# NVIDIA/vid2vid

Measured on AMD Instinct MI355X. Metric: synthesized frames/sec (Vid2VidModelG.inference, 512x256), higher is better.
Workload: dtype bf16; 1 GPU; label2city 512x256 inference, n_scales_spatial=1, --fg --use_instance, ngf=128 n_blocks=9 (411.3M params random-init, 2115 GFLOP/frame as dense convolutions, of which the 2 one-hot label stems (266 GFLOP dense) run as exact weight gather-sums), batch 1 per sequence, 1 sequence per GPU; launches_per_frame=113, hipgraph=True, graph_lanes=3, paired_launches=True, tile_selection=profiles/tune_cache.json, world_size=1, parallelism=replicas x1 (independent sequences, no collective), output_finite=True

## Files before the change

### include/v2v_hip.h

```cpp
#ifndef V2V_HIP_H
#define V2V_HIP_H

#include <stdint.h>

#ifdef __cplusplus
extern "C" {
#endif

#define V2V_EINVAL (-1)

#define V2V_F32  0
#define V2V_BF16 1

#define V2V_PAD_ZERO    0
#define V2V_PAD_REFLECT 1

#define V2V_ACT_NONE    0
#define V2V_ACT_RELU    1
#define V2V_ACT_LEAKY   2
#define V2V_ACT_TANH    3
#define V2V_ACT_SIGMOID 4

#define V2V_OUT_RAW_F32_NHWC 0
#define V2V_OUT_ACT_NHWC     1
// ... 17 lines not shown
    int32_t stride;
    int32_t pad;
    int32_t pad_mode;
    int32_t transposed;
    int32_t OH, OW;
    int32_t dtype;
    int32_t out_mode;
    int32_t act;
    float   act_param;
    float   out_scale;
    int32_t tile;
    int32_t* fin_counter;
    const float* fin_gamma;
    const float* fin_beta;
    float*  fin_scale_shift;
    float*  fin_running_mean;
    float*  fin_running_var;
    float   fin_eps;
    float   fin_momentum;
    int64_t fin_count;
    int32_t splitk;
    int32_t prefetch;
    void*   slabs;
    int32_t* sk_counter;
    int32_t w_korder;
    int32_t ablate;
    const void* res0;
    const void* res1;
    int32_t act_split;
    int32_t act_b;
    float   act_param_b;
    float   out_scale_b;
    double* fin_workspace;
} v2v_conv_desc;


#define V2V_FIN_TAG_WORD (256 + 64 * 128 + 256)




int64_t v2v_conv_packed_elems(int32_t cin, int32_t cin_stride, int32_t cout, int32_t KH, int32_t KW,
                              int32_t transposed, int32_t stride, int32_t pad, int32_t dtype);
int     v2v_conv_pack_weights(const float* w, void* dst, int32_t cin, int32_t cin_stride, int32_t cout,
                              int32_t KH, int32_t KW, int32_t transposed, int32_t stride, int32_t pad,
                              int32_t dtype, int32_t korder, void* stream);

int     v2v_conv_stats_rows(const v2v_conv_desc* d);
int     v2v_conv_stats_rows_per_sample(const v2v_conv_desc* d);
int64_t v2v_conv_splitk_workspace(const v2v_conv_desc* d, int32_t* tickets);
int     v2v_conv_fused_norm_max_workgroups(void);
int     v2v_fastdiv_magic(uint32_t d, uint32_t* m_out, int32_t* l_out);
int     v2v_conv_tile_config(const v2v_conv_desc* d);
#define V2V_TILE_FAMILY_IGEMM   0
#define V2V_TILE_FAMILY_PATCH   1
#define V2V_TILE_FAMILY_PP      2
#define V2V_TILE_FAMILY_PP2     3
#define V2V_TILE_FAMILY_PP3     4
#define V2V_TILE_FAMILY_S7      5
#define V2V_TILE_FAMILY_S2      6
#define V2V_TILE_FAMILY_T2      7
#define V2V_TILE_FAMILY_ONE     8
#define V2V_TILE_FAMILY_T2_ONE  9
#define V2V_TILE_FAMILY_HEAD    10
#define V2V_TILE_FAMILY_C8      11
#define V2V_TILE_FAMILY_ROWSUM  12
#define V2V_TILE_GROUPED        1
// ... 341 lines not shown
```

### vid2vid_amd/csrc/conv3x3_t2_kernel.h

```cpp
#pragma once
#include "conv3x3_pp3_kernel.h"

namespace v2v {

namespace t2k {
constexpr int CLS[9] = {3, 3, 3, 3, 1, 1, 2, 2, 0};
constexpr int KK[9]  = {0, 2, 6, 8, 3, 5, 1, 7, 4};
constexpr int DY[9]  = {1, 1, 0, 0, 0, 0, 1, 0, 0};
constexpr int DX[9]  = {1, 0, 1, 0, 1, 0, 0, 0, 0};
}

template <typename T, int TH, int TW, int BN, int D>
__global__ __launch_bounds__(512) void conv3x3_t2_kernel(const ConvKArgs p) {
    constexpr int VEC = ElemTraits<T>::VEC;
    constexpr int NW = 8, WGM = 4, WGN = 2, SS = 4;
    constexpr int BM = TH * TW;
    constexpr int PW = TW + 1, PR = (TH + 1) * PW;
    constexpr int NG = (PR + 7) / 8;
    constexpr int GP = (NG + NW - 1) / NW;
    constexpr int PATCH = GP * NW * 1024;
    constexpr int BST = BN * 128;
    constexpr int LB = BN / 8 / NW;
    constexpr int NPT = 9 - D;
    constexpr int PPT = (GP + NPT - 1) / NPT;
// ... 180 lines not shown
        static_for<NDMA - DMA_IN_SLOTS>([&](auto dc) { dma(std::integral_constant<int, DMA_IN_SLOTS + decltype(dc)::value>{}); });
        wait_vmcnt<pp3::pending_at(TAP, GP, LB, D)>();
        asm volatile("s_waitcnt lgkmcnt(0)" ::: "memory");
        stage = nstage;
        if constexpr (TAP == 8) {
            ++cc;
            const char* t = pa; pa = pn; pn = const_cast<char*>(t);
        }
    };
    auto chunk = [&](auto par0c) {
        constexpr int P0 = decltype(par0c)::value;
        iteration(std::integral_constant<int, 0>{}, std::integral_constant<int, P0>{});
        iteration(std::integral_constant<int, 1>{}, std::integral_constant<int, 1 - P0>{});
        iteration(std::integral_constant<int, 2>{}, std::integral_constant<int, P0>{});
        iteration(std::integral_constant<int, 3>{}, std::integral_constant<int, 1 - P0>{});
        iteration(std::integral_constant<int, 4>{}, std::integral_constant<int, P0>{});
        iteration(std::integral_constant<int, 5>{}, std::integral_constant<int, 1 - P0>{});
        iteration(std::integral_constant<int, 6>{}, std::integral_constant<int, P0>{});
        iteration(std::integral_constant<int, 7>{}, std::integral_constant<int, 1 - P0>{});
        iteration(std::integral_constant<int, 8>{}, std::integral_constant<int, P0>{});
    };
    int c = 0;
    for (; c + 1 < ncc; c += 2) {
        chunk(std::integral_constant<int, 0>{});
        chunk(std::integral_constant<int, 1>{});
    }
    if (c < ncc) chunk(std::integral_constant<int, 0>{});
    (void)nsteps;

    asm volatile("s_waitcnt vmcnt(0)" ::: "memory");
    __syncthreads();

    const int OH = p.OH, OW = p.OW;
    static_for<4>([&](auto cc_) {
        constexpr int CL = decltype(cc_)::value;
        auto pix_of = [&](int row) -> int {
            const int oy = 2 * (a0 + row / TW) + (CL >> 1), ox = 2 * (b0 + (row & (TW - 1))) + (CL & 1);
            if (oy >= OH || ox >= OW) return -1;
            return (n_img * OH + oy) * OW + ox;
        };
        conv_epilogue<T, BM, BN, WGM, WGN, false>(p, acc[CL], smem, tid, wm, wn, false, CL, tiles, lin, 0, 1, nt, CL * p.m_tiles + mt, pix_of);
        __syncthreads();
    });
}

template <typename T, int TH, int TW, int BN, int D>
static int launch_t2_cfg(const ConvKArgs& k, hipStream_t s) {
    constexpr int NW = 8;
    constexpr int GP = (((TH + 1) * (TW + 1) + 7) / 8 + NW - 1) / NW;
    const size_t lds = (size_t)2 * GP * NW * 1024 + (size_t)D * BN * 128;
    auto kern = conv3x3_t2_kernel<T, TH, TW, BN, D>;
    static bool attr_done = false;
    if (!attr_done) {
        (void)hipFuncSetAttribute(reinterpret_cast<const void*>(kern), hipFuncAttributeMaxDynamicSharedMemorySize, (int)lds);
        attr_done = true;
    }
    dim3 grid((unsigned)(k.m_tiles * k.n_tiles), 1u, 1u);
    hipLaunchKernelGGL(kern, grid, dim3(NW * 64), lds, s, k);
    return check_launch();
}

template <typename T>
static inline int launch_t2_typed(int cfg, const ConvKArgs& k, hipStream_t s) {
    switch (cfg) {
        case 110: return launch_t2_cfg<T, V2V_TILE_GEOM(110), 4>(k, s);
        case 111: return launch_t2_cfg<T, V2V_TILE_GEOM(111), 4>(k, s);
        case 112: return launch_t2_cfg<T, V2V_TILE_GEOM(112), 4>(k, s);
        case 113: return launch_t2_cfg<T, V2V_TILE_GEOM(113), 3>(k, s);
    }
    set_error("conv: unknown transposed stride-2 patch tile config %d", cfg);
    return V2V_EINVAL;
}

}
// ... 1 lines not shown
```

### vid2vid_amd/csrc/conv_igemm.hip

```cpp
#include "conv3x3_pp_kernel.h"
#include "conv3x3_pp2_kernel.h"
#include "conv3x3_pp3_kernel.h"
#include "conv3x3_s2_kernel.h"
#include "conv3x3_t2_kernel.h"
#include "conv7x7_head_kernel.h"
#include <cstdarg>
#include <cstring>
#include <cstdlib>
#include <algorithm>

namespace v2v {

static int bke_of(int dtype) { return dtype == V2V_BF16 ? 64 : 32; }

static void convt_axis(int K, int pad, int stride, int par, int* k0, int* nk, int* d0) {
    if (stride == 1) { *k0 = 0; *nk = K; *d0 = pad; return; }
    *k0 = (par + pad) & 1;
    *nk = (*k0 < K) ? (K - *k0 + 1) / 2 : 0;
    *d0 = (par + pad - *k0) / 2;
}

struct ConvGeom {
    int ncls;
    int nkh[4], nkw[4], kh0[4], kw0[4], dh0[4], dw0[4], ktot[4], kpad[4];
// ... 516 lines not shown
        break;
    case V2V_TILE_FAMILY_HEAD:
        if (d->transposed || d->KH != 7 || d->KW != 7 || d->stride != 1 || d->pad != 3 || d->cout > 32 ||
            d->cin_stride % (bke_of(d->dtype) / 2) != 0 || d->w_korder != 0 || d->splitk > 1 || d->fin_counter ||
            !(d->out_mode == V2V_OUT_F32_NCHW || d->out_mode == V2V_OUT_RAW_F32_NHWC) ||
            (d->stats && d->out_mode != V2V_OUT_RAW_F32_NHWC) || in_bytes >= (1ll << 32)) {
            set_error("conv: tile config 60 (7x7, cout <= 32) needs a 7x7/s1/p3 Conv2d, cin_stride %% %d == 0 (whole 64-byte half chunks), planar fp32 or raw "
                      "NHWC output without in-kernel norm finalize", bke_of(d->dtype) / 2); return V2V_EINVAL;
        }
        break;
    case V2V_TILE_FAMILY_S7:
        if (d->transposed || d->KH != 7 || d->KW != 7 || d->stride != 1 || d->pad != 3 ||
            d->cin_stride % bke_of(d->dtype) != 0 || d->w_korder != 1 || d->out_mode == V2V_OUT_NORM_ACT_NHWC ||
            (d->pad_mode == V2V_PAD_REFLECT && (d->H <= 3 || d->W <= 3)) || in_bytes >= (1ll << 32)) {
            set_error("conv: tile config %d needs a bf16 7x7/s1/p3 Conv2d, cin_stride %% %d == 0, korder-1 weights, no fused norm",
                      t->id, bke_of(d->dtype)); return V2V_EINVAL;
        }
        break;
    case V2V_TILE_FAMILY_T2: case V2V_TILE_FAMILY_T2_ONE:
        if (!d->transposed || d->KH != 3 || d->KW != 3 || d->stride != 2 || d->pad != 1 ||
            d->cin_stride % bke_of(d->dtype) != 0 || d->w_korder != 2 || d->splitk > 1 || d->out_mode == V2V_OUT_NORM_ACT_NHWC ||
            in_bytes >= (1ll << 32)) {
            set_error("conv: transposed stride-2 patch tile config %d needs a ConvTranspose2d(3x3, s2, p1), cin_stride %% %d == 0, korder-2 weights, no split-K",
                      t->id, bke_of(d->dtype)); return V2V_EINVAL;
        }
        if (fam == V2V_TILE_FAMILY_T2_ONE && (d->cin_stride != 64 || d->cout > t->bn || (d->cout & 3) || (d->cout_stride & 3) || ((unsigned long long)d->out & 15ull) ||
                               (d->out_mode != V2V_OUT_RAW_F32_NHWC && d->out_mode != V2V_OUT_RAW_ACT_NHWC) || d->fin_workspace != nullptr || d->H % t->th != 0 || d->W % t->tw != 0 ||
                               d->OH != 2 * d->H || d->OW != 2 * d->W)) {
            set_error("conv: tile config %d (persistent transposed stride-2 tile) needs bf16, cin_stride 64, cout <= %d and %% 4 == 0, raw fp32 NHWC output (16-byte aligned "
                      "rows), no two-level finalize workspace, H %% %d == 0, W %% %d == 0, OH = 2 H, OW = 2 W", t->id, t->bn, t->th, t->tw);
            return V2V_EINVAL;
        }
        k.woff[0] = 0; k.wrow[0] = 9 * d->cin_stride;
        k.fin_rows = (t->flags & V2V_TILE_PERSISTENT) ? 0 : 4 * k.m_tiles;
        break;
    case V2V_TILE_FAMILY_S2:
        if (d->transposed || d->KH != 3 || d->KW != 3 || d->stride != 2 || d->pad != 1 || d->pad_mode != V2V_PAD_ZERO ||
            d->cin_stride % bke_of(d->dtype) != 0 || d->w_korder != 1 || d->splitk > 1 || d->out_mode == V2V_OUT_NORM_ACT_NHWC ||
            in_bytes >= (1ll << 32)) {
            set_error("conv: stride-2 patch tile config %d needs a 3x3/s2/p1 zero-padded Conv2d, cin_stride %% %d == 0, korder-1 weights, no split-K",
                      t->id, bke_of(d->dtype)); return V2V_EINVAL;
        }
        break;
    case V2V_TILE_FAMILY_PATCH: case V2V_TILE_FAMILY_PP: case V2V_TILE_FAMILY_PP2: case V2V_TILE_FAMILY_PP3: case V2V_TILE_FAMILY_ONE: {
        const bool pad2_ok = d->pad == 2 && (t->flags & V2V_TILE_PAD2) && d->pad_mode == V2V_PAD_ZERO && d->out_mode != V2V_OUT_NORM_ACT_NHWC;
        if (d->transposed || d->KH != 3 || d->KW != 3 || d->stride != 1 || (d->pad != 1 && !pad2_ok) ||
            d->cin_stride % bke_of(d->dtype) != 0 || d->w_korder != 1 || in_bytes >= (1ll << 32)) {
            set_error("conv: patch tile config %d needs a 3x3/s1/p1 Conv2d, cin_stride %% %d == 0 and korder-1 weights",
                      t->id, bke_of(d->dtype)); return V2V_EINVAL;
        }
        if (fam == V2V_TILE_FAMILY_ONE && (((t->flags & V2V_TILE_EXACT_BN) && d->cout != t->bn) || d->cout > t->bn || (d->cout & 3) || (d->cout_stride & 3) || ((unsigned long long)d->out & 15ull) ||
                               (d->out_mode != V2V_OUT_RAW_F32_NHWC && d->out_mode != V2V_OUT_RAW_ACT_NHWC) || d->fin_workspace != nullptr || d->OH % t->th != 0 || d->OW % t->tw != 0)) {
            set_error("conv: tile configs 140 - 143 (persistent, weights resident) need cout <= %d (143: exactly) and %% 4 == 0, raw fp32 NHWC output (16-byte aligned rows), "
                      "no two-level finalize workspace, OH %% %d == 0 and OW %% %d == 0", t->bn, t->th, t->tw);
            return V2V_EINVAL;
        }
        if ((t->flags & V2V_TILE_SINGLE_CHUNK) && (d->cin_stride != bke_of(d->dtype) || d->splitk > 1 || d->out_mode == V2V_OUT_NORM_ACT_NHWC)) {
            set_error("conv: tile config %d is a single-chunk tile: bf16, cin_stride exactly %d, no split-K, no fused norm", t->id, bke_of(d->dtype));
            return V2V_EINVAL;
        }
        break;
    }
    default:
        if (d->w_korder != 0) { set_error("conv: tile config %d reads tap-major (korder 0) weights", t->id); return V2V_EINVAL; }
    }
    if (fam != V2V_TILE_FAMILY_IGEMM && k.tiles_h > 0 && k.tiles_w > 0 && k.m_tiles > 0) {
        const uint32_t dv[3] = {(uint32_t)k.m_tiles, (uint32_t)(k.tiles_h * k.tiles_w), (uint32_t)k.tiles_w};
        for (int i = 0; i < 3; ++i) {
            uint32_t m = 0; int32_t l = 0;
            if (v2v_fastdiv_magic(dv[i], &m, &l) != 0) return V2V_EINVAL;
            k.idx_m[i] = m; k.idx_l[i] = l;
        }
    }
    k.splitk = d->splitk > 1 ? d->splitk : 1;
    int nk_min = k.kpad[0] / bke_of(d->dtype);
    for (int cc = 1; cc < g.ncls; ++cc) nk_min = std::min(nk_min, k.kpad[cc] / bke_of(d->dtype));
    if (fam != V2V_TILE_FAMILY_IGEMM) nk_min = 2 * (d->cin_stride / bke_of(d->dtype));
    if (k.splitk > 1 && (k.splitk > 16 || nk_min / k.splitk < 2)) {
        set_error("conv: splitk %d needs >= 2 K chunks per slice (layer has %d)", k.splitk, nk_min); return V2V_EINVAL;
    }
    op->sk_tickets = g.ncls * k.m_tiles * k.n_tiles;
    op->slab_bytes = k.splitk > 1 ? (long long)op->sk_tickets * k.splitk * t->bm * t->bn * 4 : 0;
    if (k.splitk > 1) {
        if (launching && (!d->slabs || !d->sk_counter)) { set_error("conv: splitk needs slabs and sk_counter"); return V2V_EINVAL; }
        k.slabs = (float*)d->slabs; k.sk_counter = d->sk_counter;
    }
    if (d->fin_counter && d->fin_workspace && d->out_mode != V2V_OUT_NORM_ACT_NHWC) {
        const int rows = k.fin_rows > 0 ? k.fin_rows : g.ncls * k.m_tiles;
        const int groups = rows > 512 ? (rows >= 64 * 128 ? 64 : (rows + 127) / 128) : 0;
        if (groups > 0) {
            if (k.n_tiles > 128) { set_error("conv: two-level finalize supports up to 128 channel tiles"); return V2V_EINVAL; }
            k.fin_groups = groups; k.fin_ws = d->fin_workspace;
        }
    }
    k.ablate = d->ablate;
    k.dbg = g_conv_dbg_clocks;
    {
        static const int rev = [] { const char* e = getenv("V2V_CLS_ORDER"); return (e && e[0] == '0') ? 0 : 1; }();
        k.cls_rev = rev;
    }
    k.pf_dist = (d->prefetch > 0 && (t->flags & V2V_TILE_HELPER)) ? d->prefetch : 0;
    {
        static const int ep_fast = [] { const char* e = getenv("V2V_EPILOGUE_FAST"); return (e && e[0] == '0') ? 0 : 1; }();
        k.ep_slow = ep_fast ? 0 : 1;
    }
    k.pf_mask = (k.pf_dist > 0 && k.m_tiles >= 8) ? 3 : 0;
    return 0;
}

}

using namespace v2v;

extern "C" int64_t v2v_conv_packed_elems(int32_t cin, int32_t cin_stride, int32_t cout, int32_t KH, int32_t KW,
                                         int32_t transposed, int32_t stride, int32_t pad, int32_t dtype) {
    (void)cin;
    ConvGeom g;
    conv_geom(cin_stride, cout, KH, KW, transposed, stride, pad, dtype, &g);
    return g.total;
}

extern "C" int v2v_conv_pack_weights(const float* w, void* dst, int32_t cin, int32_t cin_stride, int32_t cout,
                                     int32_t KH, int32_t KW, int32_t transposed, int32_t stride, int32_t pad,
                                     int32_t dtype, int32_t korder, void* stream) {
    if (!w || !dst) { set_error("pack: null pointer"); return V2V_EINVAL; }
// ... 18 lines not shown
    conv_geom(cin_stride, cout, KH, KW, (korder == 4 || korder == 5) ? 0 : transposed, stride, pad, dtype, &g);
    int kh0_flip = -1;
    if (korder == 4) { kh0_flip = KH - 1; korder = 1; }
    if (korder == 5) { kh0_flip = KH - 1; korder = 0; }
    if (korder == 2) {
        g.ncls = 1; g.nkh[0] = 3; g.nkw[0] = 3; g.kh0[0] = 0; g.kw0[0] = 0;
        g.ktot[0] = g.kpad[0] = g.wrow[0] = 9 * cin_stride; g.woff[0] = 0;
        g.total = (long long)g.cout_p * g.wrow[0];
        stride = 1;
        korder = 1;
    }
    auto op = std::make_unique<PackOp>();
    PackArgs& a = op->a;
    a.w = w; a.dst = dst; a.cin = cin; a.cin_stride = cin_stride; a.cout = cout; a.cout_p = g.cout_p;
    a.KH = KH; a.KW = KW; a.transposed = transposed; a.kstep = stride; a.ncls = g.ncls; a.total = g.total; a.dtype = dtype;
    a.korder = korder; a.bke = bke_of(dtype); a.src_cl = src_cl;
    for (int c = 0; c < 4; ++c) {
        a.nkh[c] = g.nkh[c]; a.nkw[c] = g.nkw[c]; a.kh0[c] = g.kh0[c]; a.kw0[c] = g.kw0[c];
        a.kpad[c] = g.kpad[c]; a.wrow[c] = g.wrow[c]; a.woff[c] = g.woff[c];
    }
    if (kh0_flip >= 0) { a.kh0[0] = kh0_flip; a.kw0[0] = KW - 1; a.kstep = -1; }
    return submit(std::move(op), stream);
}

extern "C" int v2v_conv_debug_clocks(void* device_buffer) {
    g_conv_dbg_clocks = reinterpret_cast<unsigned long long*>(device_buffer);
    return 0;
}

extern "C" int v2v_conv_stats_rows(const v2v_conv_desc* d) {
    ConvOp op;
    if (build_conv(d, &op, false) != 0) return V2V_EINVAL;
    if (op.tile->flags & V2V_TILE_PERSISTENT) return one_grid(op.k.m_tiles * op.k.n_tiles, device_cus());
    return op.ncls * op.k.m_tiles;
}

extern "C" int v2v_conv_stats_rows_per_sample(const v2v_conv_desc* d) {
    ConvOp op;
    if (build_conv(d, &op, false) != 0) return V2V_EINVAL;
    if ((op.tile->flags & V2V_TILE_PERSISTENT) || op.ncls != 1 || d->N <= 0) return 0;
    if (op.tile->family == V2V_TILE_FAMILY_IGEMM) {
        const long long hw = (long long)d->OH * d->OW;
        return hw % op.tile->bm == 0 ? (int)(hw / op.tile->bm) : 0;
    }
    return op.k.m_tiles / d->N;
}

extern "C" int64_t v2v_conv_splitk_workspace(const v2v_conv_desc* d, int32_t* tickets) {
    ConvOp op;
    if (build_conv(d, &op, false) != 0) return V2V_EINVAL;
    if (tickets) *tickets = op.sk_tickets;
    return op.slab_bytes;
}

extern "C" int v2v_conv_tile_count(void) { return kNumConvTiles; }

extern "C" int v2v_conv_tile_info(int32_t index, struct v2v_conv_tile_info* out) {
    if (index < 0 || index >= kNumConvTiles || !out) { set_error("conv tile info: index %d outside [0, %d)", index, kNumConvTiles); return V2V_EINVAL; }
    const ConvTile& t = kConvTiles[index];
    *out = {t.id, t.family, t.bm, t.bn, t.th, t.tw, t.korder, t.flags};
    return 0;
}

extern "C" int v2v_conv_tile_config(const v2v_conv_desc* d) {
    ConvOp op;
    if (build_conv(d, &op, false) != 0) return V2V_EINVAL;
    return op.tile->id;
}


extern "C" int v2v_fastdiv_magic(uint32_t d, uint32_t* m_out, int32_t* l_out) {
    if (d == 0 || d >= (1u << 31) || !m_out || !l_out) { set_error("fastdiv: divisor out of range"); return V2V_EINVAL; }
// ... 84 lines not shown
```

### vid2vid_amd/csrc/conv_igemm_kernel.h

```cpp
#pragma once
#include "v2v_internal.h"
#include "conv_tiles.h"

namespace v2v {

struct ConvGroupPtrs {
    const char* in; const char* w; const float* bias; char* out; float* stats;
    int* fin_counter; const float* fin_gamma; const float* fin_beta; float* fin_out; float* fin_rmean; float* fin_rvar;
    float* slabs; int* sk_counter;
    const char* res0; const char* res1;
};

struct ConvKArgs {
    const char* in;
    const char* w;
    const char* zero_page;
    const float* bias;
    char* out;
    float* stats;
    int N, H, W, cin_stride;
    int cout, cout_stride, cout_p;
    int OH, OW;
    int sm;
    int os;
    int pad_mode;
    int Mc[4], OHc[4], OWc[4];
    int m_tiles, n_tiles;
    int out_mode, act;
    float act_param, out_scale;
    int nkh[4], nkw[4];
    int dh0[4], dw0[4];
    int dstep;
    int ktot[4], kpad[4], wrow[4];
    long long woff[4];
    int* fin_counter; const float* fin_gamma; const float* fin_beta; float* fin_out;
    float* fin_rmean; float* fin_rvar;
    float fin_eps, fin_momentum; double fin_inv_count, fin_unbias;
    int splitk; float* slabs; int* sk_counter;
    int pf_dist, pf_mask;
    int tiles_h, tiles_w;
    int ablate;
    int cls_rev;
    int act_split, act_b; float act_param_b, out_scale_b;
    const char* res0; const char* res1;
    unsigned div_m[4][2]; int div_l[4][2];
    int* status;
    ConvGroupPtrs g1;
    int fin_groups; double* fin_ws;
    int fin_rows;
    unsigned long long* dbg;
    int grp_xcd;
    int ep_slow;
    unsigned idx_m[3]; int idx_l[3];
    int pair_x;
};

#ifndef V2V_STAMP_MASK
#define V2V_STAMP_MASK 0
#endif
#define V2V_STAMP(p_, k_)                                                                                                   \
    do {                                                                                                                   \
        if (((V2V_STAMP_MASK >> (k_)) & 1) && (p_).dbg != nullptr && threadIdx.x == 0)                                                                       \
            (p_).dbg[((size_t)(blockIdx.z * gridDim.y + blockIdx.y) * gridDim.x + blockIdx.x) * 8 + (k_)] = wall_clock64(); \
    } while (0)

__device__ __forceinline__ int xcd_remap(int bid, int ntot) {
    const int q = ntot >> 3, r = ntot & 7, xcd = bid & 7, idx = bid >> 3;
    return (xcd < r ? xcd * (q + 1) : r * (q + 1) + (xcd - r) * q) + idx;
}

__device__ __forceinline__ int grouped_xcd_map(int bx, int bz, int ntot, int& member) {
    const int xcd = bx & 7;
    const int idx = (bx >> 3) + bz * (ntot >> 3);
    member = xcd >> 2;
    return (xcd & 3) * (ntot >> 2) + idx;
}

__device__ __forceinline__ int fast_div(int n, unsigned M, int l) { return (int)((__umulhi(M, (unsigned)n) + (unsigned)n) >> l); }

__device__ __forceinline__ void patch_tile_index(const ConvKArgs& p, const int lin_all, int& lin, int& slice, int& nt, int& mt,
                                                 int& n_img, int& th, int& tw) {
    const int S = p.splitk;
// ... 20 lines not shown
}

template <int N> __device__ __forceinline__ void wait_vmcnt() {
    asm volatile("s_waitcnt vmcnt(%0)" ::"n"(N) : "memory");
}

__device__ __forceinline__ void mfma_results_ready() {
    asm volatile("s_nop 7\n\ts_nop 7\n\ts_nop 2" ::: "memory");
    __builtin_amdgcn_sched_barrier(0);
}

template <typename T> struct Mma;
template <> struct Mma<bf16_t> {
    typedef bf16x8 Frag;
    __device__ static __forceinline__ void run(const Frag& a, const Frag& b, f32x16& c) {
        c = __builtin_amdgcn_mfma_f32_32x32x16_bf16(a, b, c, 0, 0, 0);
    }
};
template <> struct Mma<float> {
    typedef f32x4 Frag;
    __device__ static __forceinline__ void run(const Frag& a, const Frag& b, f32x16& c) {
        c = __builtin_amdgcn_mfma_f32_32x32x2f32(a[0], b[0], c, 0, 0, 0);
        c = __builtin_amdgcn_mfma_f32_32x32x2f32(a[1], b[1], c, 0, 0, 0);
        c = __builtin_amdgcn_mfma_f32_32x32x2f32(a[2], b[2], c, 0, 0, 0);
        c = __builtin_amdgcn_mfma_f32_32x32x2f32(a[3], b[3], c, 0, 0, 0);
    }
};

template <typename T, int BM, int BN, int WGM, int WGN, bool FUSED_NORM = false, typename PixOf = void>
__device__ __forceinline__ void conv_epilogue(const ConvKArgs& p, f32x16 (&acc)[BM / WGM / 32][BN / WGN / 32], char* smem,
                                              const int tid, const int wm, const int wn, const bool helper,
                                              const int cls, const int tiles, const int lin, const int slice, const int S,
                                              const int nt, const int stat_row, PixOf pix_of, const bool tile_full = false,
                                              const unsigned fin_epoch = 0u) {
    constexpr int WM = BM / WGM, WN = BN / WGN;
    constexpr int TM = WM / 32, TN = WN / 32;
    constexpr int NW = WGM * WGN;
    const int lane = tid & 63;
    const int lr = lane & 31, hi = lane >> 5;
    if (S > 1) {
        constexpr int NT = NW * 64;
        constexpr unsigned SLAB = (unsigned)BM * BN * 4u;
        typedef __attribute__((ext_vector_type(4))) unsigned u32x4;
        const long long tile_id = (long long)cls * tiles + lin;
        char* const sbase = reinterpret_cast<char*>(p.slabs) + tile_id * (long long)S * SLAB;
        const __amdgpu_buffer_rsrc_t rsrc = __builtin_amdgcn_make_buffer_rsrc(sbase, 0, (int)(S * SLAB), 0x00020000);
        if (!helper) {
            const unsigned my = (unsigned)slice * SLAB + (unsigned)tid * 16u;
#pragma unroll
            for (int i = 0; i < TM; ++i)
#pragma unroll
                for (int j = 0; j < TN; ++j)
#pragma unroll
                    for (int q = 0; q < 4; ++q) {
                        u32x4 v;
                        v[0] = __float_as_uint(acc[i][j][4 * q + 0]); v[1] = __float_as_uint(acc[i][j][4 * q + 1]);
                        v[2] = __float_as_uint(acc[i][j][4 * q + 2]); v[3] = __float_as_uint(acc[i][j][4 * q + 3]);
                        __builtin_amdgcn_raw_buffer_store_b128(v, rsrc, my + (unsigned)(((i * TN + j) * 4 + q) * NT * 16), 0, 16);
                    }
        }
        asm volatile("s_waitcnt vmcnt(0)" ::: "memory");
        __syncthreads();
        int* flag = reinterpret_cast<int*>(smem + 16384);
        if (tid == 0) {
            int* cnt = p.sk_counter + tile_id;
            const int tk = __hip_atomic_fetch_add(cnt, 1, __ATOMIC_RELAXED, __HIP_MEMORY_SCOPE_AGENT);
            const int last = tk == S - 1 ? 1 : 0;
// ... 421 lines not shown
            for (int i = 0; i < TM; ++i)
#pragma unroll
                for (int r = 0; r < 16; ++r)
                    if (opx[i][r] >= 0) {
                        const unsigned n = (unsigned)opx[i][r] / ohow;
                        opx[i][r] = (int)(n * (unsigned)p.cout * ohow + ((unsigned)opx[i][r] - n * ohow));
                    }
        }
#pragma unroll
        for (int j = 0; j < TN; ++j) {
            const int ncol = nt * BN + wn * WN + j * 32 + lr;
            const bool nvalid = ncol < p.cout && !helper;
            const float bv = (p.bias != nullptr && nvalid) ? p.bias[ncol] : 0.f;
#pragma unroll
            for (int i = 0; i < TM; ++i)
#pragma unroll
                for (int r = 0; r < 16; ++r)
                    if (opx[i][r] >= 0 && nvalid)
                        out[(unsigned)opx[i][r] + (unsigned)ncol * ohow] = apply_act(acc[i][j][r] + bv, e_act, e_act_param) * e_out_scale;
        }
    }
    V2V_STAMP(p, 4);
    if (want_stats) {
        __syncthreads();
        if (tid < BN) {
            const int ncol = nt * BN + tid;
            if (ncol < p.cout) {
                float s1 = 0.f, s2 = 0.f;
#pragma unroll
                for (int q = 0; q < WGM; ++q) {
                    s1 += red[(q * BN + tid) * 2 + 0];
                    s2 += red[(q * BN + tid) * 2 + 1];
                }
                float* dst = p.stats + ((long long)stat_row * p.cout + ncol) * 2;
                if (p.fin_counter != nullptr) {
                    const unsigned long long bits = (unsigned long long)__float_as_uint(s1) |
                                                    ((unsigned long long)__float_as_uint(s2) << 32);
                    __hip_atomic_store(reinterpret_cast<unsigned long long*>(dst), bits, __ATOMIC_RELAXED,
                                       __HIP_MEMORY_SCOPE_AGENT);
                } else {
                    dst[0] = s1;
                    dst[1] = s2;
                }
            }
        }
        if (p.fin_counter != nullptr) {
            asm volatile("s_waitcnt vmcnt(0)" ::: "memory");
            __syncthreads();
            V2V_STAMP(p, 5);
            int* flag = reinterpret_cast<int*>(smem + 16384);
            const int total = p.fin_rows > 0 ? p.fin_rows : (int)gridDim.y * p.m_tiles;
            constexpr int NT = NW * 64;
            if (p.fin_groups > 0) {
                const int G = p.fin_groups;
                int g = (int)(((long long)stat_row * G) / total);
                while ((int)(((long long)total * (g + 1)) / G) <= stat_row) ++g;
                while ((int)(((long long)total * g) / G) > stat_row) --g;
                const int r0 = (int)(((long long)total * g) / G), r1 = (int)(((long long)total * (g + 1)) / G);
                if (tid == 0) {
                    int* cnt = p.fin_counter + 256 + g * p.n_tiles + nt;
                    const int tk = __hip_atomic_fetch_add(cnt, 1, __ATOMIC_RELAXED, __HIP_MEMORY_SCOPE_AGENT);
                    const int last = tk == (r1 - r0) - 1 ? 1 : 0;
                    if (last) __hip_atomic_store(cnt, 0, __ATOMIC_RELAXED, __HIP_MEMORY_SCOPE_AGENT);
                    *flag = last;
                }
                __syncthreads();
                if (!*flag) { V2V_STAMP(p, 6); return; }
                __syncthreads();
                double* const sh = reinterpret_cast<double*>(smem);
                constexpr int CP = NT / 4 < BN ? NT / 4 : BN;
                for (int cb = 0; cb < BN; cb += CP) {
                    const int cl = cb + tid % CP, ph = tid / CP;
                    const int ncol = nt * BN + cl;
                    if (tid < 4 * CP) {
                        double s1 = 0.0, s2 = 0.0;
                        if (ncol < p.cout) {
                            const unsigned long long* const base = reinterpret_cast<const unsigned long long*>(p.stats) + ncol;
#pragma unroll 8
                            for (int r = r0 + ph; r < r1; r += 4) {
// ... 44 lines not shown
                        sh[(ph * BN + cl) * 2 + 0] = s1;
                        sh[(ph * BN + cl) * 2 + 1] = s2;
                    }
                    __syncthreads();
                    if (tid < CP && ncol < p.cout) {
                        const double s1 = ((sh[(0 * BN + cl) * 2] + sh[(1 * BN + cl) * 2]) + sh[(2 * BN + cl) * 2]) + sh[(3 * BN + cl) * 2];
                        const double s2 = ((sh[(0 * BN + cl) * 2 + 1] + sh[(1 * BN + cl) * 2 + 1]) + sh[(2 * BN + cl) * 2 + 1]) + sh[(3 * BN + cl) * 2 + 1];
                        const double mean = s1 * p.fin_inv_count;
                        double var = s2 * p.fin_inv_count - mean * mean;
                        if (var < 0.0) var = 0.0;
                        const double invstd = 1.0 / sqrt(var + (double)p.fin_eps);
                        const double gm = p.fin_gamma ? (double)p.fin_gamma[ncol] : 1.0;
                        const double bt = p.fin_beta ? (double)p.fin_beta[ncol] : 0.0;
                        const double sc = gm * invstd;
                        p.fin_out[ncol] = (float)sc;
                        p.fin_out[p.cout + ncol] = (float)(bt - mean * sc);
                        p.fin_out[2 * p.cout + ncol] = (float)mean;
                        p.fin_out[3 * p.cout + ncol] = (float)invstd;
                        if (p.fin_rmean) p.fin_rmean[ncol] = (1.f - p.fin_momentum) * p.fin_rmean[ncol] + p.fin_momentum * (float)mean;
                        if (p.fin_rvar)  p.fin_rvar[ncol]  = (1.f - p.fin_momentum) * p.fin_rvar[ncol] + p.fin_momentum * (float)(var * p.fin_unbias);
                    }
                    __syncthreads();
                }
                V2V_STAMP(p, 6);
                return;
            }
            if (tid == 0) {
                const int tk = __hip_atomic_fetch_add(p.fin_counter + nt, 1, __ATOMIC_RELAXED, __HIP_MEMORY_SCOPE_AGENT);
                const int last = tk == total - 1 ? 1 : 0;
                if (last) __hip_atomic_store(p.fin_counter + nt, 0, __ATOMIC_RELAXED, __HIP_MEMORY_SCOPE_AGENT);
                *flag = last;
            }
            __syncthreads();
            if (*flag) {
                constexpr int PH = NT / BN;
                double* acc2 = reinterpret_cast<double*>(smem);
                const int c = tid % BN, ph = tid / BN;
                const int ncol = nt * BN + c;
                double s1 = 0.0, s2 = 0.0;
                if (ncol < p.cout && ph < PH) sum_stat_rows<16>(p.stats, (long long)ncol * 2, (long long)p.cout * 2, ph, PH, total, s1, s2);
                if (ph < PH) {
                    acc2[(ph * BN + c) * 2 + 0] = s1;
                    acc2[(ph * BN + c) * 2 + 1] = s2;
                }
                __syncthreads();
                if (ph == 0 && ncol < p.cout) {
                    s1 = 0.0; s2 = 0.0;
#pragma unroll
                    for (int q = 0; q < PH; ++q) { s1 += acc2[(q * BN + c) * 2 + 0]; s2 += acc2[(q * BN + c) * 2 + 1]; }
                    const double mean = s1 * p.fin_inv_count;
                    double var = s2 * p.fin_inv_count - mean * mean;
                    if (var < 0.0) var = 0.0;
                    const double invstd = 1.0 / sqrt(var + (double)p.fin_eps);
                    const double g = p.fin_gamma ? (double)p.fin_gamma[ncol] : 1.0;
                    const double b = p.fin_beta ? (double)p.fin_beta[ncol] : 0.0;
                    const double sc = g * invstd;
                    p.fin_out[ncol] = (float)sc;
                    p.fin_out[p.cout + ncol] = (float)(b - mean * sc);
                    p.fin_out[2 * p.cout + ncol] = (float)mean;
                    p.fin_out[3 * p.cout + ncol] = (float)invstd;
                    if (p.fin_rmean) p.fin_rmean[ncol] = (1.f - p.fin_momentum) * p.fin_rmean[ncol] + p.fin_momentum * (float)mean;
                    if (p.fin_rvar)  p.fin_rvar[ncol]  = (1.f - p.fin_momentum) * p.fin_rvar[ncol] + p.fin_momentum * (float)(var * p.fin_unbias);
                }
            }
        }
    }
    V2V_STAMP(p, 6);
// ... 310 lines not shown
```

### vid2vid_amd/engine.py

```python
import contextlib
import ctypes as C
import json
import math
import os
import sys

import torch
import torch.nn as nn

from . import lib as L
from .lib import lib, check, ConvDesc
from . import tile_search as TS
from .tile_search import (TILE_CFGS, PATCH_CFGS, S2_CFGS, T2_CFGS, S7_CFGS, ABLATION_TILES, PAIR_TILES, BWD_PATCH_TILES,
                          ONE_TILES, PERSISTENT_TILES, ONE_FIN, EXP_TILES, HEAD_TILE, C8_TILE, ROWSUM_TILE, tile_korder,
                          is_patch_tile, _flag, _cfg3)

_TORCH_DTYPE = {L.F32: torch.float32, L.BF16: torch.bfloat16}


def _ptr(t):
    return None if t is None else C.c_void_p(t.data_ptr())


_HAS_GPU = []
# ... 420 lines not shown
        self.lanes_enabled = False
        self._thrash = None
        self.pair_tune_log = {}
        self.wgrad_stream_on = os.environ.get("V2V_WGRAD_STREAM", "1") != "0"
        self._wgrad_stream = None
        self._wgrad_join_queued = False
        self.repack_async_on = os.environ.get("V2V_REPACK_ASYNC", "1") != "0"
        self._repack_event = None
        import weakref
        _ENGINES.append(weakref.ref(self))
        self.plan = None
        self.conv_log = []
        self.tile_override = {}
        for item in os.environ.get("V2V_TILE_OVERRIDE", "").split(";"):
            if ":" in item:
                k, v = item.split(":")
                self.tile_override[tuple(int(x) for x in k.split(","))] = tuple(int(x) for x in v.split(","))
        self.autotune = False
        self._tuned = {}
        self.bwd_tile_override = {}
        self._tune_alts = {}
        self._tune_wide = {}
        self._tune_cache_path = os.environ.get("V2V_TUNE_CACHE", "")
        if self._tune_cache_path and os.path.exists(self._tune_cache_path):
            try:
                with open(self._tune_cache_path) as f:
                    for k, v in json.load(f).get(str(dtype), {}).items():
                        self._tuned[tuple(int(x) for x in k.split(","))] = tuple(v)
            except (OSError, ValueError):
                pass
        self.update_running_stats = False
        self.fused_finalize = True
        self.fused_finalize2 = bool(int(os.environ.get("V2V_FIN2", "0")))
        self.last_finalized = False
        self.ablate = 0

    def empty_act(self, N, H, W, C):
        t = torch.empty((N, H, W, pad_channels(C, self.dtype)), dtype=self.tdtype, device=self.device)
        self._keep(t)
        return Act(t, C)

    def zeros_act(self, N, H, W, C):
        a = self.empty_act(N, H, W, C)
        a.t.zero_()
        return a

    def empty_f32(self, *shape):
        t = torch.empty(shape, dtype=torch.float32, device=self.device)
        self._keep(t)
        return t

    def scratch(self, name, numel, dtype=torch.float32, zero=False):
        key = (name, dtype, self._lane, self._sset)
        t = self._scratch.get(key)
        if t is None or t.numel() < numel:
            if self.plan is not None and t is not None and not self.record_only:
                raise RuntimeError("scratch '%s' must not grow while a plan is recording" % name)
            t = (torch.zeros if zero else torch.empty)(int(numel), dtype=dtype, device=self.device)
            self._scratch[key] = t
        self._keep(t)
        return t

    def reserve_scratch(self, raw_elems, stats_elems):
        self.scratch("raw", raw_elems)
        self.scratch("stats", stats_elems)

# ... 292 lines not shown
        if pc.cin != x.C:
            raise RuntimeError("conv %s: input has %d channels, layer expects %d" % (label, x.C, pc.cin))
        if raw_t:
            cs = (pc.cout + 7) // 8 * 8
            d.cout_stride = cs
            out = self.scratch("raw", (N * OH * OW * cs + 1) // 2)[:N * OH * OW * cs // 2].view(torch.bfloat16)
            d.out = out.data_ptr()
        elif out_mode == L.OUT_RAW_F32_NHWC:
            cs = (pc.cout + 3) // 4 * 4
            d.cout_stride = cs
            if out is None:
                out = self.scratch("raw", N * OH * OW * cs)
            d.out = out.data_ptr()
        elif out_mode == L.OUT_ACT_NHWC:
            if out is None:
                out = self.empty_act(N, OH, OW, pc.cout)
                if out.Cs != pc.cout:
                    out.t.zero_()
            d.cout_stride = out.Cs
            d.out = out.t.data_ptr()
        else:
            if out is None:
                out = self.empty_f32(N, pc.cout, OH, OW)
            d.cout_stride = pc.cout
            d.out = out.data_ptr()
        rows = 0
        if want_stats:
            d.stats = None
            rows = lib.v2v_conv_stats_rows(C.byref(d))
            if rows <= 0:
                check(rows or -1, "conv_stats_rows")
            st = self.scratch("stats", rows * pc.cout * 2)
            d.stats = st.data_ptr()
            two_level = bool(fin is not None and N * OH * OW > FUSE_FINALIZE_MAX_PIXELS and self.fused_finalize2 and rows > 512
                             and pc.KH != 7 and d.tile not in (HEAD_TILE, C8_TILE))
            if fin is not None and N * OH * OW > FUSE_FINALIZE_MAX_PIXELS and not two_level and not (d.tile in PERSISTENT_TILES and ONE_FIN):
                fin = None
            self.last_finalized = fin is not None
            if fin is not None:
                self._attach_finalize(d, fin[0], fin[1], N, N * OH * OW)
                if two_level:
                    d.fin_workspace = self.scratch("bn_ws", 64 * pc.cout * 2, torch.float64).data_ptr()
        if pc.bias is not None:
            self._keep(pc.bias)
        if (self.autotune and d.tile == 0 and self.plan is None and not self.record_only
                and not torch.is_grad_enabled()):
            self._tuned[tune_key], self._tune_alts[tune_key], self._tune_wide[tune_key] = self._autotune(d, want_stats, pc.cout, mod, x.Cs)
            self._save_tune_cache()
            d.tile, d.splitk, d.prefetch = self._tuned[tune_key]
            pc = self._use_korder(d, mod, x.Cs, tile_korder(d.tile))
            d.bias = None if pc.bias is None else pc.bias.data_ptr()
            if want_stats:
                rows = lib.v2v_conv_stats_rows(C.byref(d))
                d.stats = self.scratch("stats", rows * pc.cout * 2).data_ptr()
        self._splitk_workspace(d)
        self._keep(pc.buf)
        if self.per_stream:
            self.last_rows_per_sample = max(int(lib.v2v_conv_stats_rows_per_sample(C.byref(d))), 0) if want_stats else 0
        check(lib.v2v_conv2d(C.byref(d), _stream()), "conv2d " + label)
        self.label(label)
        ntaps = pc.KH * pc.KW
        if len(self.conv_log) >= 100000:
            del self.conv_log[:]
        self.conv_log.append(dict(label=label, N=N, H=H, W=W, OH=OH, OW=OW, cin=pc.cin, cout=pc.cout, tune_key=tune_key,
                                  KH=pc.KH, KW=pc.KW, stride=pc.stride, transposed=pc.transposed,
                                  flops=2.0 * N * (H * W if pc.transposed else OH * OW) * pc.cout * pc.cin * ntaps,
                                  tile=lib.v2v_conv_tile_config(C.byref(d)), splitk=max(int(d.splitk), 1),
                                  prefetch=int(d.prefetch), convs=2 if act_b is not None else 1))
        return out, rows, (N, OH, OW)

    def _desc_common(self, x, pc, pad, pad_mode, OH, OW):
        d = ConvDesc()
        d.in_ = x.t.data_ptr(); d.w = pc.buf.data_ptr(); d.w_korder = pc.korder
        d.zero_page = self.zero_page().data_ptr()
        self._keep(self._zero_page)
        d.bias = None if pc.bias is None else pc.bias.data_ptr()
        d.N, d.H, d.W = x.N, x.H, x.W
        d.cin, d.cin_stride, d.cout = pc.cin, x.Cs, pc.cout
        d.KH, d.KW, d.stride, d.pad, d.pad_mode = pc.KH, pc.KW, pc.stride, pad, pad_mode
        d.transposed = int(pc.transposed)
        d.OH, d.OW = OH, OW
        d.dtype, d.out_mode, d.act = self.dtype, L.OUT_RAW_F32_NHWC, L.ACT_NONE
        d.act_param, d.out_scale = 0.0, 1.0
        d.ablate = self.ablate
        return d

    def _attach_finalize(self, d, norm, ss, N, count):
        gamma, beta, eps, mom, rm, rv = self._batchwide_params(norm, N)
        key = (self._lane, self._sset)
        fin_counter = self._fin_counters.get(key)
        if fin_counter is None:
            fin_counter = self._fin_counters[key] = torch.zeros(FIN_COUNTER_WORDS, dtype=torch.int32, device=self.device)
        d.fin_counter = fin_counter.data_ptr()
        d.fin_gamma = None if gamma is None else gamma.data_ptr()
        d.fin_beta = None if beta is None else beta.data_ptr()
        d.fin_scale_shift = ss.data_ptr()
        d.fin_running_mean = None if rm is None else rm.data_ptr()
        d.fin_running_var = None if rv is None else rv.data_ptr()
        d.fin_eps, d.fin_momentum, d.fin_count = eps, mom, count
        for t in (gamma, beta, ss, fin_counter):
            if t is not None:
                self._keep(t)

    def _bn_finalize(self, rows, cout, count, norm, ss, N, label):
        gamma, beta, eps, mom, rm, rv = self._batchwide_params(norm, N)
        st = self.scratch("stats", rows * cout * 2)
        for t in (gamma, beta):
            if t is not None:
                self._keep(t)
        groups = lib.v2v_bn_finalize_groups(rows)
        ws = self.scratch("bn_ws", groups * cout * 2, torch.float64) if groups > 0 else None
        check(lib.v2v_bn_finalize(_ptr(st), rows, cout, count, _ptr(gamma), _ptr(beta), eps,
                                  _ptr(ss), _ptr(rm), _ptr(rv), mom, _ptr(ws), _stream()), "bn_finalize " + label)
        self.label(label + ".norm")

    def pair_eligible(self, xa, ma, xb, mb):
        if self._training() or not isinstance(ma, nn.Conv2d) or not isinstance(mb, nn.Conv2d):
# ... 951 lines not shown
```

### vid2vid_amd/lib.py

```python
import ctypes as C
import os

_HERE = os.path.dirname(os.path.abspath(__file__))
LIB_PATH = os.environ.get("V2V_LIB_PATH") or os.path.join(_HERE, "libv2v_hip.so")

F32, BF16 = 0, 1
PAD_ZERO, PAD_REFLECT = 0, 1
ACT_NONE, ACT_RELU, ACT_LEAKY, ACT_TANH, ACT_SIGMOID = 0, 1, 2, 3, 4
OUT_RAW_F32_NHWC, OUT_ACT_NHWC, OUT_F32_NCHW, OUT_NORM_ACT_NHWC, OUT_RAW_ACT_NHWC = 0, 1, 2, 3, 4


class ConvDesc(C.Structure):
    _fields_ = [
        ("in_", C.c_void_p), ("w", C.c_void_p), ("bias", C.c_void_p), ("out", C.c_void_p),
        ("stats", C.c_void_p), ("zero_page", C.c_void_p),
        ("N", C.c_int32), ("H", C.c_int32), ("W", C.c_int32),
        ("cin", C.c_int32), ("cin_stride", C.c_int32),
        ("cout", C.c_int32), ("cout_stride", C.c_int32),
        ("KH", C.c_int32), ("KW", C.c_int32),
        ("stride", C.c_int32), ("pad", C.c_int32), ("pad_mode", C.c_int32),
        ("transposed", C.c_int32),
        ("OH", C.c_int32), ("OW", C.c_int32),
        ("dtype", C.c_int32), ("out_mode", C.c_int32), ("act", C.c_int32),
        ("act_param", C.c_float), ("out_scale", C.c_float),
        ("tile", C.c_int32),
        ("fin_counter", C.c_void_p), ("fin_gamma", C.c_void_p), ("fin_beta", C.c_void_p),
        ("fin_scale_shift", C.c_void_p), ("fin_running_mean", C.c_void_p), ("fin_running_var", C.c_void_p),
        ("fin_eps", C.c_float), ("fin_momentum", C.c_float), ("fin_count", C.c_int64),
        ("splitk", C.c_int32), ("prefetch", C.c_int32), ("slabs", C.c_void_p), ("sk_counter", C.c_void_p),
        ("w_korder", C.c_int32), ("ablate", C.c_int32),
        ("res0", C.c_void_p), ("res1", C.c_void_p),
        ("act_split", C.c_int32), ("act_b", C.c_int32), ("act_param_b", C.c_float), ("out_scale_b", C.c_float),
        ("fin_workspace", C.c_void_p),
    ]


class ConvTileInfo(C.Structure):
    _fields_ = [(n, C.c_int32) for n in ("id", "family", "bm", "bn", "th", "tw", "korder", "flags")]


(TILE_IGEMM, TILE_PATCH, TILE_PP, TILE_PP2, TILE_PP3, TILE_S7, TILE_S2, TILE_T2, TILE_ONE, TILE_T2_ONE, TILE_HEAD, TILE_C8,
 TILE_ROWSUM) = range(13)
(TILE_GROUPED, TILE_FUSED_NORM, TILE_PAD2, TILE_SINGLE_CHUNK, TILE_PERSISTENT, TILE_HELPER, TILE_BF16_ONLY, TILE_ABLATION,
 TILE_EXPERIMENT, TILE_EXACT_BN) = (1 << i for i in range(10))


class OneHotNorm(C.Structure):
    _fields_ = [
        ("counter", C.c_void_p), ("gamma", C.c_void_p), ("beta", C.c_void_p), ("scale_shift", C.c_void_p),
        ("running_mean", C.c_void_p), ("running_var", C.c_void_p), ("eps", C.c_float), ("momentum", C.c_float),
        ("count", C.c_int64),
    ]


class WgradDesc(C.Structure):
    _fields_ = [
        ("p", C.c_void_p), ("q", C.c_void_p), ("grad", C.c_void_p), ("workspace", C.c_void_p), ("zero_page", C.c_void_p),
        ("N", C.c_int32), ("OH", C.c_int32), ("OW", C.c_int32), ("QH", C.c_int32), ("QW", C.c_int32),
        ("rows", C.c_int32), ("cols", C.c_int32), ("p_stride", C.c_int32), ("q_stride", C.c_int32),
        ("KH", C.c_int32), ("KW", C.c_int32), ("stride", C.c_int32), ("pad", C.c_int32), ("pad_mode", C.c_int32),
        ("dtype", C.c_int32), ("accumulate", C.c_int32),
    ]


LOSS_MSE_CONST, LOSS_L1 = 0, 1
FACE_DENSEPOSE, FACE_OPENPOSE = 0, 1
# ... 172 lines not shown
```

Baseline: 395.3 frames/s.

## Fuse BN finalize into conv launch for small stat-row counts; add T2 one-row stats

Lets conv launches with at most a configurable number of stat rows (default 512) run the batch-norm finalize inside the same launch, using a new ordered four-phase reduction path. It also adds an opt-in mode where the transposed stride-2 kernel accumulates its four parity classes into one stats row per tile. The aim is to drop separate finalize launches and cut stats-row traffic. The cost is extra last-block reduction work and a different summation order, and the one-row mode is off by default.

```diff
diff --git a/include/v2v_hip.h b/include/v2v_hip.h
--- a/include/v2v_hip.h
+++ b/include/v2v_hip.h
@@ -73,7 +73,9 @@
     float   act_param_b;
     float   out_scale_b;
     double* fin_workspace;
+    int32_t stats_one_row;
 } v2v_conv_desc;
+
 
 
 #define V2V_FIN_TAG_WORD (256 + 64 * 128 + 256)
diff --git a/vid2vid_amd/csrc/conv3x3_t2_kernel.h b/vid2vid_amd/csrc/conv3x3_t2_kernel.h
--- a/vid2vid_amd/csrc/conv3x3_t2_kernel.h
+++ b/vid2vid_amd/csrc/conv3x3_t2_kernel.h
@@ -236,6 +236,7 @@
     __syncthreads();
 
     const int OH = p.OH, OW = p.OW;
+    float carry[2] = {0.f, 0.f};
     static_for<4>([&](auto cc_) {
         constexpr int CL = decltype(cc_)::value;
         auto pix_of = [&](int row) -> int {
@@ -243,7 +244,8 @@
             if (oy >= OH || ox >= OW) return -1;
             return (n_img * OH + oy) * OW + ox;
         };
-        conv_epilogue<T, BM, BN, WGM, WGN, false>(p, acc[CL], smem, tid, wm, wn, false, CL, tiles, lin, 0, 1, nt, CL * p.m_tiles + mt, pix_of);
+        if (p.one_row) conv_epilogue<T, BM, BN, WGM, WGN, false>(p, acc[CL], smem, tid, wm, wn, false, CL, tiles, lin, 0, 1, nt, mt, pix_of, false, 0u, carry, CL < 3);
+        else           conv_epilogue<T, BM, BN, WGM, WGN, false>(p, acc[CL], smem, tid, wm, wn, false, CL, tiles, lin, 0, 1, nt, CL * p.m_tiles + mt, pix_of);
         __syncthreads();
     });
 }
diff --git a/vid2vid_amd/csrc/conv_igemm.hip b/vid2vid_amd/csrc/conv_igemm.hip
--- a/vid2vid_amd/csrc/conv_igemm.hip
+++ b/vid2vid_amd/csrc/conv_igemm.hip
@@ -572,7 +572,8 @@
             return V2V_EINVAL;
         }
         k.woff[0] = 0; k.wrow[0] = 9 * d->cin_stride;
-        k.fin_rows = (t->flags & V2V_TILE_PERSISTENT) ? 0 : 4 * k.m_tiles;
+        k.one_row = (fam == V2V_TILE_FAMILY_T2 && d->stats_one_row) ? 1 : 0;
+        k.fin_rows = ((t->flags & V2V_TILE_PERSISTENT) || k.one_row) ? 0 : 4 * k.m_tiles;
         break;
     case V2V_TILE_FAMILY_S2:
         if (d->transposed || d->KH != 3 || d->KW != 3 || d->stride != 2 || d->pad != 1 || d->pad_mode != V2V_PAD_ZERO ||
@@ -626,11 +627,13 @@
         k.slabs = (float*)d->slabs; k.sk_counter = d->sk_counter;
     }
     if (d->fin_counter && d->fin_workspace && d->out_mode != V2V_OUT_NORM_ACT_NHWC) {
-        const int rows = k.fin_rows > 0 ? k.fin_rows : g.ncls * k.m_tiles;
+        const int rows = k.one_row ? k.m_tiles : k.fin_rows > 0 ? k.fin_rows : g.ncls * k.m_tiles;
         const int groups = rows > 512 ? (rows >= 64 * 128 ? 64 : (rows + 127) / 128) : 0;
         if (groups > 0) {
             if (k.n_tiles > 128) { set_error("conv: two-level finalize supports up to 128 channel tiles"); return V2V_EINVAL; }
             k.fin_groups = groups; k.fin_ws = d->fin_workspace;
+        } else {
+            k.fin_bn_order = 1;
         }
     }
     k.ablate = d->ablate;
@@ -715,12 +718,14 @@
     ConvOp op;
     if (build_conv(d, &op, false) != 0) return V2V_EINVAL;
     if (op.tile->flags & V2V_TILE_PERSISTENT) return one_grid(op.k.m_tiles * op.k.n_tiles, device_cus());
+    if (op.k.one_row) return op.k.m_tiles;
     return op.ncls * op.k.m_tiles;
 }
 
 extern "C" int v2v_conv_stats_rows_per_sample(const v2v_conv_desc* d) {
     ConvOp op;
     if (build_conv(d, &op, false) != 0) return V2V_EINVAL;
+    if (op.k.one_row && d->N > 0) return op.k.m_tiles / d->N;
     if ((op.tile->flags & V2V_TILE_PERSISTENT) || op.ncls != 1 || d->N <= 0) return 0;
     if (op.tile->family == V2V_TILE_FAMILY_IGEMM) {
         const long long hw = (long long)d->OH * d->OW;
diff --git a/vid2vid_amd/csrc/conv_igemm_kernel.h b/vid2vid_amd/csrc/conv_igemm_kernel.h
--- a/vid2vid_amd/csrc/conv_igemm_kernel.h
+++ b/vid2vid_amd/csrc/conv_igemm_kernel.h
@@ -48,6 +48,8 @@
     ConvGroupPtrs g1;
     int fin_groups; double* fin_ws;
     int fin_rows;
+    int one_row;
+    int fin_bn_order;
     unsigned long long* dbg;
     int grp_xcd;
     int ep_slow;
@@ -134,7 +136,7 @@
                                               const int tid, const int wm, const int wn, const bool helper,
                                               const int cls, const int tiles, const int lin, const int slice, const int S,
                                               const int nt, const int stat_row, PixOf pix_of, const bool tile_full = false,
-                                              const unsigned fin_epoch = 0u) {
+                                              const unsigned fin_epoch = 0u, float* const carry = nullptr, const bool carry_hold = false) {
     constexpr int WM = BM / WGM, WN = BN / WGN;
     constexpr int TM = WM / 32, TN = WN / 32;
     constexpr int NW = WGM * WGN;
@@ -622,8 +624,13 @@
                     s1 += red[(q * BN + tid) * 2 + 0];
                     s2 += red[(q * BN + tid) * 2 + 1];
                 }
+                if (carry != nullptr) {
+                    s1 = carry[0] + s1; s2 = carry[1] + s2;
+                    carry[0] = s1; carry[1] = s2;
+                }
                 float* dst = p.stats + ((long long)stat_row * p.cout + ncol) * 2;
-                if (p.fin_counter != nullptr) {
+                if (carry_hold) {
+                } else if (p.fin_counter != nullptr) {
                     const unsigned long long bits = (unsigned long long)__float_as_uint(s1) |
                                                     ((unsigned long long)__float_as_uint(s2) << 32);
                     __hip_atomic_store(reinterpret_cast<unsigned long long*>(dst), bits, __ATOMIC_RELAXED,
@@ -634,7 +641,7 @@
                 }
             }
         }
-        if (p.fin_counter != nullptr) {
+        if (p.fin_counter != nullptr && !carry_hold) {
             asm volatile("s_waitcnt vmcnt(0)" ::: "memory");
             __syncthreads();
             V2V_STAMP(p, 5);
@@ -745,7 +752,39 @@
                 *flag = last;
             }
             __syncthreads();
-            if (*flag) {
+            if (*flag && p.fin_bn_order) {
+                double* const sh = reinterpret_cast<double*>(smem);
+                constexpr int CP = NT / 4 < BN ? NT / 4 : BN;
+                for (int cb = 0; cb < BN; cb += CP) {
+                    const int cl = cb + tid % CP, ph = tid / CP;
+                    const int ncol = nt * BN + cl;
+                    if (tid < 4 * CP) {
+                        double s1 = 0.0, s2 = 0.0;
+                        if (ncol < p.cout) sum_stat_rows<16>(p.stats, (long long)ncol * 2, (long long)p.cout * 2, ph, 4, total, s1, s2);
+                        sh[(ph * BN + cl) * 2 + 0] = s1;
+                        sh[(ph * BN + cl) * 2 + 1] = s2;
+                    }
+                    __syncthreads();
+                    if (tid < CP && ncol < p.cout) {
+                        const double s1 = ((sh[(0 * BN + cl) * 2] + sh[(1 * BN + cl) * 2]) + sh[(2 * BN + cl) * 2]) + sh[(3 * BN + cl) * 2];
+                        const double s2 = ((sh[(0 * BN + cl) * 2 + 1] + sh[(1 * BN + cl) * 2 + 1]) + sh[(2 * BN + cl) * 2 + 1]) + sh[(3 * BN + cl) * 2 + 1];
+                        const double mean = s1 * p.fin_inv_count;
+                        double var = s2 * p.fin_inv_count - mean * mean;
+                        if (var < 0.0) var = 0.0;
+                        const double invstd = 1.0 / sqrt(var + (double)p.fin_eps);
+                        const double gm = p.fin_gamma ? (double)p.fin_gamma[ncol] : 1.0;
+                        const double bt = p.fin_beta ? (double)p.fin_beta[ncol] : 0.0;
+                        const double sc = gm * invstd;
+                        p.fin_out[ncol] = (float)sc;
+                        p.fin_out[p.cout + ncol] = (float)(bt - mean * sc);
+                        p.fin_out[2 * p.cout + ncol] = (float)mean;
+                        p.fin_out[3 * p.cout + ncol] = (float)invstd;
+                        if (p.fin_rmean) p.fin_rmean[ncol] = (1.f - p.fin_momentum) * p.fin_rmean[ncol] + p.fin_momentum * (float)mean;
+                        if (p.fin_rvar)  p.fin_rvar[ncol]  = (1.f - p.fin_momentum) * p.fin_rvar[ncol] + p.fin_momentum * (float)(var * p.fin_unbias);
+                    }
+                    __syncthreads();
+                }
+            } else if (*flag) {
                 constexpr int PH = NT / BN;
                 double* acc2 = reinterpret_cast<double*>(smem);
                 const int c = tid % BN, ph = tid / BN;
diff --git a/vid2vid_amd/engine.py b/vid2vid_amd/engine.py
--- a/vid2vid_amd/engine.py
+++ b/vid2vid_amd/engine.py
@@ -476,6 +476,8 @@
         self.update_running_stats = False
         self.fused_finalize = True
         self.fused_finalize2 = bool(int(os.environ.get("V2V_FIN2", "0")))
+        self.fin_max_rows = int(os.environ.get("V2V_FIN_ROWS", "512"))
+        self.t2_one_row = bool(int(os.environ.get("V2V_T2_ONE_ROW", "0")))
         self.last_finalized = False
         self.ablate = 0
 
@@ -834,14 +836,16 @@
                 check(rows or -1, "conv_stats_rows")
             st = self.scratch("stats", rows * pc.cout * 2)
             d.stats = st.data_ptr()
-            two_level = bool(fin is not None and N * OH * OW > FUSE_FINALIZE_MAX_PIXELS and self.fused_finalize2 and rows > 512
-                             and pc.KH != 7 and d.tile not in (HEAD_TILE, C8_TILE))
-            if fin is not None and N * OH * OW > FUSE_FINALIZE_MAX_PIXELS and not two_level and not (d.tile in PERSISTENT_TILES and ONE_FIN):
+            big = N * OH * OW > FUSE_FINALIZE_MAX_PIXELS
+            can_fin = d.tile not in (HEAD_TILE, C8_TILE) and (pc.KH != 7 or d.tile != 0)
+            in_launch = bool(fin is not None and big and can_fin and d.tile not in PERSISTENT_TILES
+                             and (rows <= self.fin_max_rows or (self.fused_finalize2 and rows > 512)))
+            if fin is not None and big and not in_launch and not (d.tile in PERSISTENT_TILES and ONE_FIN):
                 fin = None
             self.last_finalized = fin is not None
             if fin is not None:
                 self._attach_finalize(d, fin[0], fin[1], N, N * OH * OW)
-                if two_level:
+                if in_launch:
                     d.fin_workspace = self.scratch("bn_ws", 64 * pc.cout * 2, torch.float64).data_ptr()
         if pc.bias is not None:
             self._keep(pc.bias)
@@ -885,6 +889,7 @@
         d.dtype, d.out_mode, d.act = self.dtype, L.OUT_RAW_F32_NHWC, L.ACT_NONE
         d.act_param, d.out_scale = 0.0, 1.0
         d.ablate = self.ablate
+        d.stats_one_row = int(self.t2_one_row)
         return d
 
     def _attach_finalize(self, d, norm, ss, N, count):
diff --git a/vid2vid_amd/lib.py b/vid2vid_amd/lib.py
--- a/vid2vid_amd/lib.py
+++ b/vid2vid_amd/lib.py
@@ -32,6 +32,7 @@
         ("res0", C.c_void_p), ("res1", C.c_void_p),
         ("act_split", C.c_int32), ("act_b", C.c_int32), ("act_param_b", C.c_float), ("out_scale_b", C.c_float),
         ("fin_workspace", C.c_void_p),
+        ("stats_one_row", C.c_int32),
     ]
 
 
```

Result: slower. 390.4 frames/s (-1.3%).
